# yuliangguo/OmniFusion

Measured on AMD Instinct MI355X. Metric: panoramas/sec at 512x1024 ERP, N=18 256^2 patches; equi2pers+pers2equi GB/s vs HBM peak, higher is better.
Workload: dtype f16x3 (fp16 hi/lo pairs, fp32 accumulate: fp32-class); 1 GPU; cfg2/cfg4 shard: 8 panoramas/GPU/step, 512x1024 ERP, fov 80, nrows 4 (18 patches); full single-pass spherical_fusion forward (confidence=True) at patch size 128 — the only size the reference network exists at (SURVEY 0.1); random-init weights (seed 42); inputs resident in HBM; resample pair at 18x256^2 reported in roofline_resample; per_gpu_batch=8, global_batch=8, parallelism=image-sharded x1, execution=3 forwards in flight per GPU on 3 streams (spherical_fusion.pipelined)

## Files before the change

omnifusion_amd/csrc/omni_conv_sh.hip:

```cpp
#include "omni_conv_sh_common.h"

namespace {

__constant__ float wino_coef[16][4] = {
    {1, 0, 0, 0}, {1, 1, 0, 0}, {1, -1, 0, 0}, {0, -1, 0, 0},
    {1, 0, 1, 0}, {1, 1, 1, 1}, {1, -1, 1, -1}, {0, -1, 0, -1},
    {1, 0, -1, 0}, {1, 1, -1, -1}, {1, -1, -1, 1}, {0, -1, 0, 1},
    {0, 0, -1, 0}, {0, 0, -1, -1}, {0, 0, -1, 1}, {0, 0, 0, 1}};
template <int BM, int BN, int WM, int WN, int NST = 3, int NL = 0, bool PP = false, bool WINO = false, bool X1 = false>
__global__ __launch_bounds__(64 * (WM * WN + NL)) void conv_sh_kernel(ShConvArgs a)
{
    static_assert(!(WINO && X1), "Winograd: f16x3 only");
    static_assert(!PP || (NL > 0 && WM * WN == 8 && NST >= 3), "ping-pong: eight matrix waves (two per SIMD) + loader waves, three stages");
    static_assert(!WINO || (PP && BM / WM == 32 && BN / WN == 32), "Winograd: the ping-pong kernel with 32 x 32 wave tiles");
    constexpr int NW = WM * WN, LW = NL > 0 ? NL : NW, RPP = 8 * LW;
    constexpr int TM = BM / WM / 32, TN = BN / WN / 32;
    constexpr int APASS = BM / RPP, BPASS = BN / RPP, LPS = APASS + BPASS;
    static_assert(APASS >= 1 && BPASS >= 1, "a tile side must cover at least one DMA pass");
    constexpr int A_BYTES = BM * 128, STAGE = (BM + BN) * 128;
    __shared__ __attribute__((aligned(1024))) unsigned char lds[NST * STAGE];
    __shared__ long long cst[OMNI_ABL(32768) ? 256 : 1];
    const bool stamped = OMNI_ABL(32768) && blockIdx.x == 0 && blockIdx.y == 0 && a.ws != nullptr && a.splitk <= 1;
    auto cstamp = [&](int k) { if (OMNI_ABL(32768) && stamped && (threadIdx.x & 63) == 0 && k < 256) cst[k] = clock64(); };
    auto cdump = [&]() { if (OMNI_ABL(32768) && stamped && threadIdx.x == 0) for (int i = 0; i < 256; ++i) reinterpret_cast<long long*>(a.ws)[i] = cst[i]; };
// ... 498 lines not shown
                                       const void* res, void* dst, int fmt, int M, int H, int W, int C1, int C2, int Cout,
                                       int KH, int KW, int stride, int pad, int act, int splitk, float* ws, size_t ws_bytes,
                                       omni_stream_t stream)
{
    return conv2d_sh_impl(src1, src2, wt16, bias, res, dst, fmt, M, H, W, C1, C2, Cout, KH, KW, stride, pad, act, splitk, ws, ws_bytes,
                          nullptr, 0, stream);
}
extern "C" int omni_conv2d_sh_f16x3_post_ws(const void* src1, const void* src2, const void* wt16, const float* bias,
                                            const void* res, void* dst, int fmt, int M, int H, int W, int C1, int C2, int Cout,
                                            int KH, int KW, int stride, int pad, int act, int splitk, float* ws, size_t ws_bytes,
                                            const float* post, size_t post_elems, omni_stream_t stream)
{
    return conv2d_sh_impl(src1, src2, wt16, bias, res, dst, fmt, M, H, W, C1, C2, Cout, KH, KW, stride, pad, act, splitk, ws, ws_bytes,
                          post, post_elems, stream);
}
extern "C" int omni_gemm_sh_f16x3_ln512_ws(const void* x, const void* wt16, const float* bias, const float* res, float* tok, const float* ln_g, const float* ln_b,
                                           float eps, void* y, int fmt, int rows, int K, int splitk, float* ws, size_t ws_bytes, omni_stream_t stream)
{
    if (!x || !wt16 || !tok || !ln_g || !ln_b || !y) OMNI_FAIL(OMNI_ERR_INVALID, "omni_gemm_sh_f16x3_ln512: null pointer");
    if (rows <= 0 || K <= 0 || K % 32) OMNI_FAIL(OMNI_ERR_INVALID, "omni_gemm_sh_f16x3_ln512: bad shape");
    if (fmt & 8) OMNI_FAIL(OMNI_ERR_UNSUPPORTED, "omni_gemm_sh_f16x3_ln512: no f16x1 form (fmt bit 3)");
    const int S = std::min(splitk, K / 32);
    if (S < 2) OMNI_FAIL(OMNI_ERR_INVALID, "omni_gemm_sh_f16x3_ln512: needs a split-K plan (splitk >= 2); an unsplit GEMM writes its result in its own epilogue");
    const int rc = conv2d_sh_impl(x, nullptr, wt16, bias, res, tok, 2, rows, 1, 1, K, 0, 512, 1, 1, 1, 0, OMNI_ACT_NONE, S, ws, ws_bytes, nullptr, 0, stream, false);
    if (rc != OMNI_OK) return rc;
    hipStream_t s = (hipStream_t)stream;
    if (fmt & 1) hipLaunchKernelGGL(sh_splitk_reduce_ln512_kernel<true>, dim3((rows + 3) / 4), dim3(256), 0, s, (const float*)ws, bias, res, tok, ln_g, ln_b, y, rows, S, (size_t)rows * 512, eps);
    else         hipLaunchKernelGGL(sh_splitk_reduce_ln512_kernel<false>, dim3((rows + 3) / 4), dim3(256), 0, s, (const float*)ws, bias, res, tok, ln_g, ln_b, y, rows, S, (size_t)rows * 512, eps);
    OMNI_HIP(hipGetLastError());
    return OMNI_OK;
}

constexpr int OMNI_HALO2_MIN_BLOCKS = 256;
template <bool X1>
static void conv_sh_select(const ShConvArgs& a, int fmt, hipStream_t s)
{
    const int KH = a.KH, KW = a.KW, stride = a.stride, pad = a.pad, H = a.H, W = a.W, M = a.M, Cout = a.Cout;
    const int ksteps = KH * KW * ((a.C1 + a.C2) / 32);
    const long long rows = a.rows;
    if (const int h2 = omni_options().conv_halo2; h2 > 0 && a.splitk <= 1 && KH == 3 && KW == 3 && stride == 1 && pad == 1 && Cout % 64 == 0 && rows % 256 == 0 &&
        !(fmt & 4) && !omni_options().conv_nohalo && omni_options().conv_halo_bn != 32) {
        const int iw = (H == 16 && W == 16 && omni_options().conv_img > 0) ? 16 : (W % HT_W == 0 && H % 8 == 0) ? 0 : -1;
        const long long blocks = (rows / 256) * (Cout / 64);
        if (iw >= 0 && (h2 == 2 || blocks >= (h2 == 1 ? OMNI_HALO2_MIN_BLOCKS : h2))) { omni_halo2_launch(&a, iw, X1, s); return; }
    }
    if (a.splitk <= 1 && KH == 3 && KW == 3 && stride == 1 && pad == 1 && H == W && (W == 16 || (W == 8 && omni_options().conv_img >= 2)) && rows % 128 == 0 &&
        Cout % 64 == 0 && !(fmt & 4) && omni_options().conv_img > 0 && !omni_options().conv_nohalo) {
        const int grid = (int)(rows / 128) * (Cout / 64);
        if (omni_options().conv_halo_bn == 32) {
            if (W == 16) omni_halo_launch(&a, 32, 4, false, 16, X1, 2 * grid, s);
            else         omni_halo_launch(&a, 32, 4, false, 8, X1, 2 * grid, s);
        }
        else if (W == 16) omni_halo_launch(&a, 64, 4, false, 16, X1, grid, s);
        else         omni_halo_launch(&a, 64, 4, false, 8, X1, grid, s);
        return;
    }
    if (a.splitk <= 1 && KH == 3 && KW == 3 && stride == 1 && pad == 1 && W % HT_W == 0 && H % 4 == 0 && !omni_options().conv_nohalo) {
        const int th = (H % 8 == 0 && omni_options().conv_halo_th == 8) ? 8 : 4;
        const int grid = M * (H / th) * (W / HT_W);
        if (th == 8) {
            if (Cout % 64 == 0 && omni_options().conv_halo_bn != 32) omni_halo_launch(&a, 64, 8, false, 0, X1, grid * (Cout / 64), s);
            else                omni_halo_launch(&a, 32, 8, false, 0, X1, grid * (Cout / 32), s);
        } else {
            const bool bn32 = omni_options().conv_halo_bn == 32 || ((fmt & 4) && omni_options().conv_halo_bn_lat == 32);
            if (Cout % 64 == 0 && !bn32) omni_halo_launch(&a, 64, 4, false, 0, X1, grid * (Cout / 64), s);
            else                omni_halo_launch(&a, 32, 4, false, 0, X1, grid * (Cout / 32), s);
        }
        return;
    }
    int tile = omni_options().conv_sh_tile;
    if (tile < 0) tile = 8;
    const int pm = omni_options().conv_pm;
    const bool pm_shape = pm > 0 && KH == 3 && KW == 3 && stride == 1 && pad == 1 && H == W && (W == 8 || W == 4) && Cout % 64 == 0 && !a.post &&
                          omni_options().conv_pingpong && !(pm == 3 && W != 8) && !(pm == 4 && W != 4);
    if (pm_shape && pm == 2) { omni_conv_pm_launch(&a, Cout % 128 == 0 ? 128 : 64, X1, s); return; }
    const bool big256 = tile == 8 && Cout % 128 == 0 && ((rows + 255) / 256) * (long long)(Cout / 128) * a.splitk >= std::max(1, omni_options().conv_big_blocks);
    if (pm_shape && tile == 8 && !big256) {
        if (Cout % 128 == 0 && ((rows + 127) / 128) * (long long)(Cout / 128) * a.splitk >= 128) { omni_conv_pm_launch(&a, 128, X1, s); return; }
        if (((rows + 127) / 128) * (long long)(Cout / 64) * a.splitk >= 128) { omni_conv_pm_launch(&a, 64, X1, s); return; }
    }
    if (Cout % 64 != 0) launch_sh<X1, 128, 32, 4, 1>(a, s);
    else if (tile == 2 && Cout % 128 == 0) launch_sh<X1, 128, 128, 2, 2>(a, s);
    else if (tile == 1) launch_sh<X1, 128, 64, 2, 2>(a, s);
    else if (tile == 3) launch_sh<X1, 128, 64, 4, 2>(a, s);
    else if (tile == 4 && Cout % 128 == 0) launch_sh<X1, 128, 128, 4, 2>(a, s);
    else if (tile == 8 && Cout % 128 == 0 && ((rows + 255) / 256) * (long long)(Cout / 128) * a.splitk >= std::max(1, omni_options().conv_big_blocks)) launch_sh<X1, 256, 128, 4, 2>(a, s);
    else if (tile == 8 && Cout % 128 == 0 && ((rows + 127) / 128) * (long long)(Cout / 128) * a.splitk >= 128) launch_sh<X1, 128, 128, 4, 2, 3, 4>(a, s);
    else if (tile == 8 && ((rows + 127) / 128) * (long long)(Cout / 64) * a.splitk >= 128) launch_sh<X1, 128, 64, 4, 2, 3, 4>(a, s);
    else if (tile == 9 && Cout % 128 == 0 && ((rows + 255) / 256) * (long long)(Cout / 128) * a.splitk >= 128) launch_sh<X1, 256, 128, 4, 2>(a, s);
// ... 52 lines not shown
    hipStream_t s = (hipStream_t)stream;
    if (fmt & 8) conv_sh_select<true>(a, fmt, s);
    else         conv_sh_select<false>(a, fmt, s);
    OMNI_HIP(hipGetLastError());
    if (a.splitk > 1 && reduce) {
        const size_t n4 = (size_t)rows * Cout / 4;
        hipLaunchKernelGGL(sh_splitk_reduce_kernel, dim3((unsigned)((n4 + 255) / 256)), dim3(256), 0, s, (const float*)ws, bias, res, dst,
                           n4, Cout, a.splitk, (size_t)rows * Cout, act, a.dst_sh, a.res_f32);
        OMNI_HIP(hipGetLastError());
    }
    return OMNI_OK;
}

extern "C" int omni_splitk_reduce_ln512(const float* parts, int nparts, const float* bias, const float* res, float* tok, const float* lg, const float* lb,
                                        float eps, void* y, int fmt, int rows, omni_stream_t stream)
{
    if (!parts || nparts < 1 || !tok || !lg || !lb || !y || rows <= 0) OMNI_FAIL(OMNI_ERR_INVALID, "omni_splitk_reduce_ln512: null pointer or empty input");
    hipStream_t s = (hipStream_t)stream;
    if (fmt & 1) hipLaunchKernelGGL(sh_splitk_reduce_ln512_kernel<true>, dim3((rows + 3) / 4), dim3(256), 0, s, parts, bias, res, tok, lg, lb, y, rows, nparts, (size_t)rows * 512, eps);
    else         hipLaunchKernelGGL(sh_splitk_reduce_ln512_kernel<false>, dim3((rows + 3) / 4), dim3(256), 0, s, parts, bias, res, tok, lg, lb, y, rows, nparts, (size_t)rows * 512, eps);
    OMNI_HIP(hipGetLastError());
    return OMNI_OK;
}

OMNI_SH_OVERFLOW_ACCESSOR(omni_sh_overflow_conv)

extern "C" int omni_sh_overflow(int* flag, int reset)
{
    if (!flag) OMNI_FAIL(OMNI_ERR_INVALID, "omni_sh_overflow: null output");
    OMNI_HIP(hipDeviceSynchronize());
    unsigned v = 0;
    if (omni_sh_overflow_conv(&v, reset) != 0 || omni_sh_overflow_halo(&v, reset) != 0 || omni_sh_overflow_up2(&v, reset) != 0 ||
        omni_sh_overflow_rows(&v, reset) != 0 || omni_sh_overflow_net(&v, reset) != 0 || omni_sh_overflow_pm(&v, reset) != 0 ||
        omni_sh_overflow_halo2(&v, reset) != 0)
        OMNI_FAIL(OMNI_ERR_HIP, "omni_sh_overflow: could not read the device flag");
    *flag = v ? 1 : 0;
    return OMNI_OK;
}

extern "C" int omni_sh_from_f32(const float* src, void* dst, size_t n, omni_stream_t stream)
{
    if (!src || !dst || n % 32) OMNI_FAIL(OMNI_ERR_INVALID, "omni_sh_from_f32: null pointer or n % 32 != 0");
    if (n == 0) return OMNI_OK;
    hipLaunchKernelGGL(sh_from_f32_kernel, dim3((unsigned)((n / 4 + 255) / 256)), dim3(256), 0, (hipStream_t)stream, src, dst, n / 4);
    OMNI_HIP(hipGetLastError());
    return OMNI_OK;
}
extern "C" int omni_sh_to_f32(const void* src, float* dst, size_t n, omni_stream_t stream)
{
    if (!src || !dst || n % 32) OMNI_FAIL(OMNI_ERR_INVALID, "omni_sh_to_f32: null pointer or n % 32 != 0");
    if (n == 0) return OMNI_OK;
    hipLaunchKernelGGL(sh_to_f32_kernel, dim3((unsigned)((n / 4 + 255) / 256)), dim3(256), 0, (hipStream_t)stream, src, dst, n / 4);
    OMNI_HIP(hipGetLastError());
    return OMNI_OK;
}

namespace {

__global__ __launch_bounds__(256) void wino_input_sh_kernel(const void* __restrict__ src, void* __restrict__ V, int M, int H, int W, int C, size_t nt)
{
    const size_t i = (size_t)blockIdx.x * 256 + threadIdx.x;
    const int cq = C >> 2;
    if (i >= nt * cq) return;
    const size_t tl = i / cq;
    const int c = (int)(i - tl * cq) * 4;
    const int tw = W >> 1, th = H >> 1;
    const int m = (int)(tl / (size_t)(th * tw)), rem = (int)(tl - (size_t)m * th * tw), ty = rem / tw, tx = rem - ty * tw;
// ... 63 lines not shown
```

omnifusion_amd/csrc/omni_conv_sh_common.h:

```cpp
#pragma once
#include <stdlib.h>
#include <algorithm>
#include <type_traits>
#include "omni_internal.h"
#include "omni_sh.h"

#ifndef OMNI_CONV_ABL
#define OMNI_CONV_ABL 0
#endif
#define OMNI_ABL(bit) ((OMNI_CONV_ABL & (bit)) != 0)
#ifndef OMNI_PP_PRIO
#define OMNI_PP_PRIO 0
#endif
#ifndef OMNI_G1_PW
#define OMNI_G1_PW 4
#endif

namespace {

typedef float f16v __attribute__((ext_vector_type(16)));
typedef float f4v __attribute__((ext_vector_type(4)));
typedef _Float16 h8v __attribute__((ext_vector_type(8)));
typedef _Float16 h4v __attribute__((ext_vector_type(4)));
typedef _Float16 h2v __attribute__((ext_vector_type(2)));
// ... 171 lines not shown

__device__ __forceinline__ void splitk_finish(f4v v, size_t o, const float* __restrict__ bias, const void* __restrict__ res, void* __restrict__ dst,
                                              int Cout, int act, int dst_sh, int res_f32)
{
    if (bias) v += *reinterpret_cast<const f4v*>(bias + (o % Cout));
    if (res && res_f32) v += *reinterpret_cast<const f4v*>((const float*)res + o);
    else if (res) {
        const unsigned char* rp = (const unsigned char*)res + sh_off(o);
        v += sh_join4(*reinterpret_cast<const h4v*>(rp), *reinterpret_cast<const h4v*>(rp + 64));
    }
    if (act == OMNI_ACT_RELU) { v.x = fmaxf(v.x, 0.f); v.y = fmaxf(v.y, 0.f); v.z = fmaxf(v.z, 0.f); v.w = fmaxf(v.w, 0.f); }
    else if (act == OMNI_ACT_GELU) {
#pragma unroll
        for (int e = 0; e < 4; ++e) v[e] = 0.5f * v[e] * (1.0f + erff(v[e] * 0.70710678118654752440f));
    }
    if (dst_sh) {
        h4v hi, lo; sh_split4(v, hi, lo);
        unsigned char* dp = (unsigned char*)dst + sh_off(o);
        *reinterpret_cast<h4v*>(dp) = hi; *reinterpret_cast<h4v*>(dp + 64) = lo;
    } else {
        *reinterpret_cast<f4v*>((float*)dst + o) = v;
    }
}

constexpr int HT_W = 32, HPW = HT_W + 2;

}

void omni_halo_launch(const void* args, int bn, int th, bool up2, int iw, bool x1, unsigned grid, hipStream_t s);
void omni_conv_pm_launch(const void* args, int bn, bool x1, hipStream_t s);
int omni_sh_overflow_pm(unsigned* out, int reset);
void omni_halo2_launch(const void* args, int iw, bool x1, hipStream_t s);
int omni_sh_overflow_halo2(unsigned* out, int reset);
int omni_sh_overflow_halo(unsigned* out, int reset);
int omni_sh_overflow_up2(unsigned* out, int reset);
int omni_sh_overflow_rows(unsigned* out, int reset);
int omni_sh_overflow_net(unsigned* out, int reset);
```

omnifusion_amd/csrc/omni_conv_up2.hip:

```cpp
#include "omni_conv_sh_common.h"

namespace {

constexpr int HR_PITCH = 36;
struct HeadsArgs { const void* w16; float* hr; };

template <bool HEADS, bool X1 = false>
__global__ __launch_bounds__(HEADS ? 64 * (4 + OMNI_G1_PW) : 512) void conv3x3_up2_g1_kernel(ShConvArgs a, int ntiles, HeadsArgs hd)
{
    constexpr int BN = 32, TH = 4, NW = 4, RPP = 8 * NW;
    constexpr int PW = HEADS ? OMNI_G1_PW : 4, CPT = 32 / PW;
    constexpr int HPX = (TH + 2) * HPW, HA_INSTR = (HPX * 8 + 63) / 64, HA_BYTES = HA_INSTR * 1024;
    constexpr int BROWS = 3 * BN, BPASS = (BROWS + RPP - 1) / RPP, B_BYTES = BROWS * 128, W_OFF = 2 * HA_BYTES;
    __shared__ __attribute__((aligned(1024))) unsigned char lds[2 * HA_BYTES + 3 * B_BYTES];
    constexpr int ST_N = 40, ST_K = 5;
    __shared__ long long stamps[OMNI_ABL(32768) ? 2 * ST_N * ST_K : 1];
    auto stamp = [&](int who, int it, int k) { if (OMNI_ABL(32768) && blockIdx.x == 0 && it < ST_N && (threadIdx.x & 63) == 0) stamps[(who * ST_N + it) * ST_K + k] = clock64(); };

    const int t = threadIdx.x, lane = t & 63;
    const int wave = __builtin_amdgcn_readfirstlane(t >> 6);
    const bool consumer = wave < NW;
    const int tw = a.W / HT_W, th = a.H / TH, per_img = tw * th;
    const int xcd = blockIdx.x & 7, lb = blockIdx.x >> 3, nlb = gridDim.x >> 3;
    const int per = (ntiles + 7) >> 3, t_end = min(ntiles, (xcd + 1) * per);
// ... 266 lines not shown
}

}

OMNI_SH_OVERFLOW_ACCESSOR(omni_sh_overflow_up2)

extern "C" int omni_conv3x3_up2_sh_f16x3(const void* src, const void* wt16, const float* bias, void* dst, int fmt,
                                         int M, int Hl, int Wl, int C, int Cout, int act, omni_stream_t stream)
{
    if (!src || !wt16 || !dst) OMNI_FAIL(OMNI_ERR_INVALID, "omni_conv3x3_up2_sh: null pointer");
    if (M <= 0 || Hl <= 0 || Wl <= 0 || C <= 0 || C % 32 || Cout <= 0 || Cout % 32) OMNI_FAIL(OMNI_ERR_INVALID, "omni_conv3x3_up2_sh: bad shape (channels must be multiples of 32)");
    const int H = 2 * Hl, W = 2 * Wl;
    if (W % HT_W || H % 4) OMNI_FAIL(OMNI_ERR_UNSUPPORTED, "omni_conv3x3_up2_sh: the output must be a multiple of 4 rows x 32 columns");
    if ((long long)M * H * W >= (1ll << 31) || (long long)Cout * 9 * C * 4 >= (1ll << 31))
        OMNI_FAIL(OMNI_ERR_UNSUPPORTED, "omni_conv3x3_up2_sh: tensor too large for 32-bit indices");
    ShConvArgs a;
    a.src1 = src; a.src2 = nullptr; a.wt = wt16; a.bias = bias; a.res = nullptr; a.dst = dst; a.dst_sh = fmt & 1; a.res_f32 = 0;
    a.dbg = 0; a.noxcd = omni_options().conv_noxcd; a.wt_major = 0; a.epi_lds = omni_options().conv_epi_lds && !(fmt & 4);
#ifdef OMNI_DEBUG_BUILD
    a.dbg = omni_debug_bits("OMNI_CONV_DBG");
#endif
    a.M = M; a.H = H; a.W = W; a.C1 = C; a.C2 = 0; a.Cout = Cout; a.KH = 3; a.KW = 3; a.stride = 1; a.pad = 1; a.act = act;
    a.Ho = H; a.Wo = W; a.rows = M * H * W; a.splitk = 1; a.ws = nullptr; a.post = nullptr; a.post_rows = 1; a.wino_th = a.wino_tw = a.wino_pix = 0;
    const int grid = M * (H / 4) * (W / HT_W);
    const bool x1 = (fmt & 8) != 0;
    if (C == 32 && Cout == 32 && omni_options().conv_up2_persist) {
        const dim3 g1(grid < 256 ? (grid + 7) / 8 * 8 : 256);
        if (x1) hipLaunchKernelGGL((conv3x3_up2_g1_kernel<false, true>), g1, dim3(512), 0, (hipStream_t)stream, a, grid, HeadsArgs{nullptr, nullptr});
        else    hipLaunchKernelGGL(conv3x3_up2_g1_kernel<false>, g1, dim3(512), 0, (hipStream_t)stream, a, grid, HeadsArgs{nullptr, nullptr});
        OMNI_HIP(hipGetLastError());
        return OMNI_OK;
    }
    const bool bn64 = Cout % 64 == 0 && !((fmt & 4) && omni_options().conv_halo_up2_bn_lat == 32);
    if (bn64) omni_halo_launch(&a, 64, 4, true, 0, x1, grid * (Cout / 64), (hipStream_t)stream);
    else      omni_halo_launch(&a, 32, 4, true, 0, x1, grid * (Cout / 32), (hipStream_t)stream);
    OMNI_HIP(hipGetLastError());
    return OMNI_OK;
}

extern "C" size_t omni_up2_heads_scratch_bytes(int M, int P)
{
    if (M <= 0 || P <= 0 || P % 32) return 0;
    return (size_t)M * (P / 4) * (P / 32) * 4 * 6 * HR_PITCH * sizeof(float);
}
template <bool X1>
static int up2_heads_impl(const void* src, const void* wt16, const float* bias, const void* heads_w16f, float bias_pred, float bias_weight,
                          float* scratch, size_t scratch_bytes, float* out_a, float* out_c, int M, int P, int confidence, omni_stream_t stream)
{
    if (!src || !wt16 || !heads_w16f || !scratch || !out_a) OMNI_FAIL(OMNI_ERR_INVALID, "omni_conv3x3_up2_heads_sh: null pointer");
    if (M <= 0 || P <= 0 || P % 32) OMNI_FAIL(OMNI_ERR_INVALID, "omni_conv3x3_up2_heads_sh: the patch size must be a multiple of 32");
    if (scratch_bytes < omni_up2_heads_scratch_bytes(M, P)) OMNI_FAIL(OMNI_ERR_INVALID, "omni_conv3x3_up2_heads_sh: scratch too small (omni_up2_heads_scratch_bytes)");
    if ((long long)M * P * P >= (1ll << 31)) OMNI_FAIL(OMNI_ERR_UNSUPPORTED, "omni_conv3x3_up2_heads_sh: tensor too large for 32-bit indices");
    ShConvArgs a;
    a.src1 = src; a.src2 = nullptr; a.wt = wt16; a.bias = bias; a.res = nullptr; a.dst = nullptr; a.dst_sh = 0; a.res_f32 = 0;
    a.dbg = 0; a.noxcd = omni_options().conv_noxcd; a.wt_major = 0; a.epi_lds = 0;
    a.M = M; a.H = P; a.W = P; a.C1 = 32; a.C2 = 0; a.Cout = 32; a.KH = 3; a.KW = 3; a.stride = 1; a.pad = 1; a.act = OMNI_ACT_RELU;
    a.Ho = P; a.Wo = P; a.rows = M * P * P; a.splitk = 1; a.ws = nullptr; a.post = nullptr; a.post_rows = 1; a.wino_th = a.wino_tw = a.wino_pix = 0;
    const int grid = M * (P / 4) * (P / HT_W);
    hipLaunchKernelGGL((conv3x3_up2_g1_kernel<true, X1>), dim3(grid < 256 ? (grid + 7) / 8 * 8 : 256), dim3(64 * (4 + OMNI_G1_PW)), 0, (hipStream_t)stream, a, grid, HeadsArgs{heads_w16f, scratch});
    OMNI_HIP(hipGetLastError());
    const size_t n = (size_t)M * P * P / 4;
    hipLaunchKernelGGL(heads_finish_kernel, dim3((unsigned)((n + 255) / 256)), dim3(256), 0, (hipStream_t)stream, (const float*)scratch, bias_pred, bias_weight,
                       out_a, out_c, M, P, confidence);
    OMNI_HIP(hipGetLastError());
    return OMNI_OK;
}
extern "C" int omni_conv3x3_up2_heads_sh_f16x3(const void* src, const void* wt16, const float* bias, const void* heads_w16f, float bias_pred, float bias_weight,
// ... 30 lines not shown
```

omnifusion_amd/csrc/omni_geometry.hip:

```cpp
#include <math.h>
#include <stdlib.h>
#include <string.h>
#include <mutex>
#include <vector>
#include <memory>

#include "omni_internal.h"

static thread_local std::string g_err;
void omni_set_error(const std::string& msg) { g_err = msg; }
extern "C" const char* omni_last_error(void) { return g_err.c_str(); }
extern "C" int omni_version(void) { return OMNI_VERSION; }

namespace {
struct OptName { const char* name; const char* env; int OmniOptions::* field; int dflt; };
const OptName kOpts[] = {
    {"conv_sh_tile", "OMNI_CONV_SH_TILE", &OmniOptions::conv_sh_tile, -1},
    {"conv_nohalo", "OMNI_CONV_NOHALO", &OmniOptions::conv_nohalo, 0},
    {"conv_halo_th", "OMNI_CONV_HALO_TH", &OmniOptions::conv_halo_th, 4},
    {"conv_big_blocks", "OMNI_CONV_BIG_BLOCKS", &OmniOptions::conv_big_blocks, 128},
    {"conv_halo_bn_lat", "OMNI_CONV_HALO_BN_LAT", &OmniOptions::conv_halo_bn_lat, 32},
    {"conv_deep_loaders", "OMNI_CONV_DEEP_LOADERS", &OmniOptions::conv_deep_loaders, 1},
    {"conv_halo_up2_bn_lat", "OMNI_CONV_HALO_UP2_BN_LAT", &OmniOptions::conv_halo_up2_bn_lat, 64},
    {"conv_halo_bn", "OMNI_CONV_HALO_BN", &OmniOptions::conv_halo_bn, 64},
// ... 11 lines not shown
    {"e2p_notab", "OMNI_E2P_NOTAB", &OmniOptions::e2p_notab, 0},
    {"e2p_verbose", "OMNI_E2P_VERBOSE", &OmniOptions::e2p_verbose, 0},
    {"e2p_bwd_simple", "OMNI_E2P_BWD_SIMPLE", &OmniOptions::e2p_bwd_simple, 0},
    {"p2e_bwd_simple", "OMNI_P2E_BWD_SIMPLE", &OmniOptions::p2e_bwd_simple, 0},
    {"bwd_table_mb", "OMNI_BWD_TABLE_MB", &OmniOptions::bwd_table_mb, 1024},
    {"bwd_wide", "OMNI_BWD_WIDE", &OmniOptions::bwd_wide, 1},
    {"bwd_lmax", "OMNI_BWD_LMAX", &OmniOptions::bwd_lmax, 0},
    {"bwd_chunk", "OMNI_BWD_CHUNK", &OmniOptions::bwd_chunk, 0},
    {"p2e_gather", "OMNI_P2E_GATHER", &OmniOptions::p2e_gather, 0},
    {"e2p_nbuf", "OMNI_E2P_NBUF", &OmniOptions::e2p_nbuf, 0},
    {"e2p_slot_kb", "OMNI_E2P_SLOT_KB", &OmniOptions::e2p_slot_kb, 6},
    {"e2p_tile_h", "OMNI_E2P_TILE_H", &OmniOptions::e2p_tile_h, 0},
    {"e2p_ref_lds", "OMNI_E2P_REF_LDS", &OmniOptions::e2p_ref_lds, 1},
    {"e2p_store", "OMNI_E2P_STORE", &OmniOptions::e2p_store, 1},
    {"e2p_slots", "OMNI_E2P_SLOTS", &OmniOptions::e2p_slots, 0},
    {"e2p_split", "OMNI_E2P_SPLIT", &OmniOptions::e2p_split, 0},
    {"e2p_full", "OMNI_E2P_FULL", &OmniOptions::e2p_full, -1},
    {"e2p_fb_planes", "OMNI_E2P_FB_PLANES", &OmniOptions::e2p_fb_planes, 0},
    {"e2p_fb_pos", "OMNI_E2P_FB_POS", &OmniOptions::e2p_fb_pos, 0},
    {"e2p_region", "OMNI_E2P_REGION", &OmniOptions::e2p_region, 0},
    {"p2e_band", "OMNI_P2E_BAND", &OmniOptions::p2e_band, 0},
    {"p2e_nbuf", "OMNI_P2E_NBUF", &OmniOptions::p2e_nbuf, 0},
    {"p2e_lds_kb", "OMNI_P2E_LDS_KB", &OmniOptions::p2e_lds_kb, 0},
    {"p2e_planes", "OMNI_P2E_PLANES", &OmniOptions::p2e_planes, 0},
    {"p2e_walk", "OMNI_P2E_WALK", &OmniOptions::p2e_walk, 1},
    {"p2e_tile8", "OMNI_P2E_TILE8", &OmniOptions::p2e_tile8, 1},
    {"p2e_store", "OMNI_P2E_STORE", &OmniOptions::p2e_store, 1},
    {"fv_bwd_lds", "OMNI_FV_BWD_LDS", &OmniOptions::fv_bwd_lds, 1},
    {"geom_cache_max", "OMNI_GEOM_CACHE_MAX", &OmniOptions::geom_cache_max, 16},
    {"chamfer_split", "OMNI_CHAMFER_SPLIT", &OmniOptions::chamfer_split, 1},
    {"augment_lut", "OMNI_AUGMENT_LUT", &OmniOptions::augment_lut, 1},
    {"conv_halo2", "OMNI_CONV_HALO2", &OmniOptions::conv_halo2, 1},
    {"conv_wgrad_rows", "OMNI_CONV_WGRAD_ROWS", &OmniOptions::conv_wgrad_rows, 0},
};
}

OmniOptions& omni_options()
{
    static OmniOptions o = [] {
        OmniOptions v;
        for (const OptName& k : kOpts) {
            const char* e = getenv(k.env);
            v.*(k.field) = e ? (*e ? atoi(e) : 1) : k.dflt;
        }
        return v;
    }();
    return o;
}

int omni_num_cus()
{
    static int cus[64] = {0};
    int dev = 0;
    if (hipGetDevice(&dev) != hipSuccess || dev < 0 || dev >= 64) return 256;
    if (cus[dev] == 0) {
        int n = 0;
        cus[dev] = (hipDeviceGetAttribute(&n, hipDeviceAttributeMultiprocessorCount, dev) == hipSuccess && n > 0) ? n : 256;
    }
    return cus[dev];
}

extern "C" int omni_set_option(const char* name, int value)
{
    if (!name) OMNI_FAIL(OMNI_ERR_INVALID, "omni_set_option: null name");
    for (const OptName& k : kOpts)
        if (strcmp(k.name, name) == 0) { omni_options().*(k.field) = value; return OMNI_OK; }
// ... 235 lines not shown
```

omnifusion_amd/csrc/omni_internal.h:

```cpp
#pragma once
#include <mutex>
#include <hip/hip_runtime.h>
#include <hip/hip_fp16.h>
#include <stdint.h>
#include <string>
#include <vector>

#include "../../include/omnifusion.h"

#define OMNI_MAX_PATCH 46
#define OMNI_WAVE 64

void omni_set_error(const std::string& msg);
#define OMNI_FAIL(code, msg) do { omni_set_error(msg); return (code); } while (0)
#define OMNI_HIP(expr) do { hipError_t e_ = (expr); if (e_ != hipSuccess) {                   \
        omni_set_error(std::string(#expr) + ": " + hipGetErrorString(e_)); return OMNI_ERR_HIP; } } while (0)

struct OmniOptions {
    int conv_sh_tile;
    int conv_nohalo;
    int conv_halo_th;
    int conv_halo_bn_lat;
    int conv_halo_up2_bn_lat;
    int conv_deep_loaders;
// ... 13 lines not shown
    int e2p_notab;
    int e2p_verbose;
    int e2p_bwd_simple;
    int p2e_bwd_simple;
    int p2e_gather;
    int e2p_nbuf;
    int e2p_store;
    int e2p_slots;
    int e2p_split;
    int e2p_full;
    int e2p_fb_planes;
    int e2p_region;
    int e2p_fb_pos;
    int e2p_ref_lds;
    int e2p_tile_h;
    int e2p_slot_kb;
    int p2e_band;
    int p2e_lds_kb;
    int p2e_nbuf;
    int p2e_planes;
    int p2e_store;
    int p2e_tile8;
    int p2e_walk;
    int bwd_wide;
    int bwd_chunk;
    int bwd_lmax;
    int bwd_table_mb;
    int fv_bwd_lds;
    int geom_cache_max;
    int chamfer_split;
    int augment_lut;
    int conv_halo2;
    int conv_wgrad_rows;
};
OmniOptions& omni_options();
int omni_num_cus();

#ifdef OMNI_DEBUG_BUILD
#define OMNI_DBG(a, bit) (((a).dbg & (bit)) != 0)
int omni_debug_bits(const char* env_name);
long long* omni_debug_trace_buf();
#else
#define OMNI_DBG(a, bit) false
#endif

struct PatchTab {
    int   N;
    float lam0[OMNI_MAX_PATCH];
    float slam[OMNI_MAX_PATCH];
    float clam[OMNI_MAX_PATCH];
    float sphi[OMNI_MAX_PATCH];
    float cphi[OMNI_MAX_PATCH];
};

constexpr int OMNI_SP_LMAX = 48;
struct OmniSpTable {
    uint2* ent = nullptr; int* slice_off = nullptr; int* cnt = nullptr;
    uint2* long_ent = nullptr; int* long_off = nullptr; int* long_row = nullptr;
    int nrows = 0, nslices = 0, nlong = 0, ok = 0;
    long long nent = 0, npadded = 0, nlong_ent = 0;
};
void omni_sp_free(OmniSpTable& t);
struct omni_geometry;
int omni_bwd_workspace(omni_geometry* g, hipStream_t stream, size_t bytes, float** out);

struct omni_geometry {
// ... 79 lines not shown
```

omnifusion_amd/isa.py:

```python
import os
import re
import subprocess
import sys
import tempfile

LLVM = os.environ.get("OMNI_LLVM_BIN", "/opt/rocm/lib/llvm/bin")
TARGET = "hipv4-amdgcn-amd-amdhsa--gfx950"
FORBIDDEN = re.compile(r"\bv_pk_(mul|add|fma)_f32\b")
COUNTED = ("e2p_box_kernel", "p2e_lds_kernel", "p2e_walk_kernel", "e2p_ref_kernel")
HOT = ("conv_sh_kernel", "conv3x3_halo_sh_kernel", "conv3x3_up2_g1_kernel", "stem_f16x3_pc_kernel", "heads_kernel", "maxpool_kernel",
       "layernorm512_kernel", "attention_kernel", "upsample_sh8_kernel", "halo2_sh_kernel")
HOST_ONLY = ("omni_png.o", "omni_geometry.o")


def _device_object(obj, tmp):
    fat = os.path.join(tmp, "fat.bin")
    co = os.path.join(tmp, "dev.co")
    r = subprocess.run([os.path.join(LLVM, "llvm-objcopy"), "--dump-section", f".hip_fatbin={fat}", obj, os.path.join(tmp, "copy.o")],
                       stderr=subprocess.DEVNULL)
    if r.returncode != 0 or not os.path.exists(fat) or os.path.getsize(fat) == 0:
        return None
    subprocess.check_call([os.path.join(LLVM, "clang-offload-bundler"), "--unbundle", "--type=o", f"--input={fat}",
                           f"--targets={TARGET}", f"--output={co}"])
    return co


def disassemble(obj):
    with tempfile.TemporaryDirectory() as tmp:
        co = _device_object(obj, tmp)
        if co is None:
            return ""
        return subprocess.check_output([os.path.join(LLVM, "llvm-objdump"), "-d", "--mcpu=gfx950", co]).decode()


def kernel_meta(obj):
    with tempfile.TemporaryDirectory() as tmp:
        co = _device_object(obj, tmp)
        if co is None:
            return []
        txt = subprocess.check_output([os.path.join(LLVM, "llvm-readelf"), "--notes", co]).decode()
    out, cur = [], None
    keys = {".vgpr_count": "vgpr", ".agpr_count": "agpr", ".sgpr_count": "sgpr", ".group_segment_fixed_size": "lds",
            ".private_segment_fixed_size": "scratch", ".vgpr_spill_count": "vgpr_spill", ".sgpr_spill_count": "sgpr_spill",
            ".name": "name"}
# ... 88 lines not shown
```

Measured before the change: 4362 panoramas/s.

## Add 8-row halo conv kernel with fused 2x bilinear upsampling and 32-wide form

Adds a new 3x3 convolution kernel that covers 8 output rows per block. It stages the haloed input tile once per channel group in LDS and streams weights through a four-slot ring. One variant builds the upsampled input tile directly in LDS from the half-resolution source, using bilinear interpolation split into fp16 hi/lo parts. The other variant handles Cout not divisible by 64 with 32-channel tiles. Both are enabled by default through a new option and are chosen when the existing halo2 block-count heuristic allows. The aim is to raise input reuse and to avoid materialising the upsampled tensor, at the cost of more LDS and register pressure, fewer blocks, and extra interpolation math inside the kernel.

```diff
diff --git a/omnifusion_amd/csrc/omni_conv_halo2x.hip b/omnifusion_amd/csrc/omni_conv_halo2x.hip
--- /dev/null
+++ b/omnifusion_amd/csrc/omni_conv_halo2x.hip
@@ -0,0 +1,270 @@
+#include <stdio.h>
+#include <string.h>
+#include "omni_conv_sh_common.h"
+
+namespace {
+
+template <int BN, bool UP2, bool X1>
+__global__ __launch_bounds__(256, 2) void halo2x_sh_kernel(ShConvArgs a)
+{
+    static_assert((BN == 64 && UP2) || (BN == 32 && !UP2), "the up-sampling form with 64 channels per block, the copying form with 32");
+    constexpr int TN = BN / 32, NW = 4, RPP = 8 * NW, RING = 4, TROWS = 8;
+    constexpr int HPX = (TROWS + 2) * HPW, HA_INSTR = (HPX * 8 + 63) / 64, HA_BYTES = HA_INSTR * 1024;
+    constexpr int APASS = (HA_INSTR + NW - 1) / NW, BPASS = BN / RPP, B_BYTES = BN * 128;
+    constexpr int CROWS = (TROWS + 2) / 2, CCOLS = HPW / 2, UTASKS = CROWS * CCOLS * 4;
+    static_assert(UTASKS > 256 && UTASKS <= 384, "one pass of four waves and one of two");
+    __shared__ __attribute__((aligned(1024))) unsigned char lds[HA_BYTES + RING * B_BYTES];
+    static_assert(sizeof(lds) <= 80 * 1024, "two blocks per CU");
+
+    const int t = threadIdx.x, lane = t & 63;
+    const int wave = __builtin_amdgcn_readfirstlane(t >> 6);
+    const int ntn = a.Cout / BN, tw = a.W / HT_W, th = a.H / TROWS;
+    int bid = a.noxcd ? blockIdx.x : omni_xcd_remap(blockIdx.x, gridDim.x);
+    const int tile_n = bid % ntn; bid /= ntn;
+    const int tx = bid % tw; bid /= tw;
+    const int ty = bid % th; const int m = bid / th;
+    const int y0 = ty * TROWS, x0 = tx * HT_W, col0 = tile_n * BN;
+    const int G1 = a.C1 >> 5, G = (a.C1 + a.C2) >> 5, ksteps = 9 * G;
+
+    const int gs = (lane & 15) ^ ((4 * wave + (lane >> 4)) & 15);
+    const int rl = 8 * wave + 2 * (lane >> 4) + (gs >> 3), pc16 = (gs & 7) * 16;
+    int wbase[BPASS];
+#pragma unroll
+    for (int i = 0; i < BPASS; ++i) wbase[i] = (col0 + rl + RPP * i) * ksteps * 128 + pc16;
+    const rsrc_t rsw = make_rsrc(a.wt, (size_t)a.Cout * ksteps * 128);
+
+    [[maybe_unused]] auto issue_a = [&](int g) {
+        const rsrc_t rs1 = make_rsrc(a.src1, (size_t)a.M * a.H * a.W * a.C1 * 4);
+        const rsrc_t rs2 = make_rsrc(a.src2 ? a.src2 : a.src1, a.src2 ? (size_t)a.M * a.H * a.W * a.C2 * 4 : 0);
+        const bool first = g < G1;
+        const int cs4 = (first ? a.C1 : a.C2) * 4;
+        const int soff = (first ? g : g - G1) * 128 + pc16;
+        unsigned char* sb = lds + wave * 1024;
+        int rlv = rl;
+        asm volatile("" : "+v"(rlv));
+#pragma unroll
+        for (int i = 0; i < APASS; ++i) {
+            if (wave + NW * i < HA_INSTR) {
+                const int p = rlv + RPP * i, hy = p / HPW, hx = p - hy * HPW;
+                const int iy = y0 - 1 + hy, ix = x0 - 1 + hx;
+                const int px = (p < HPX && (unsigned)iy < (unsigned)a.H && (unsigned)ix < (unsigned)a.W) ? (m * a.H + iy) * a.W + ix : -1;
+                const int off = px >= 0 ? px * cs4 + soff : (int)0x80000000;
+                if (first) dma16(rs1, sb + i * (1024 * NW), off, 0);
+                else       dma16(rs2, sb + i * (1024 * NW), off, 0);
+            }
+        }
+    };
+
+    [[maybe_unused]] auto up_load = [&](int g, int task, h8v (&ch)[4], h8v (&cl)[4]) {
+        const int Hl = a.H >> 1, Wl = a.W >> 1;
+        const int u_c8 = task & 3, u_cell = task >> 2, u_ci = u_cell / CCOLS, u_cj = u_cell - u_ci * CCOLS;
+        const int u_k = (y0 >> 1) - 1 + u_ci, u_j = (x0 >> 1) - 1 + u_cj;
+        const int ra = min(max(u_k, 0), Hl - 1), rb = min(max(u_k + 1, 0), Hl - 1), ca = min(max(u_j, 0), Wl - 1), cb = min(max(u_j + 1, 0), Wl - 1);
+        const size_t pp = (size_t)a.C1 * 4, img = (size_t)m * Hl * Wl;
+        const unsigned char* sp = (const unsigned char*)a.src1 + (size_t)g * 128 + u_c8 * 16;
+        const size_t u_src[4] = {(img + (size_t)ra * Wl + ca) * pp, (img + (size_t)ra * Wl + cb) * pp, (img + (size_t)rb * Wl + ca) * pp, (img + (size_t)rb * Wl + cb) * pp};
+#pragma unroll
+        for (int q = 0; q < 4; ++q) { ch[q] = *reinterpret_cast<const h8v*>(sp + u_src[q]); cl[q] = *reinterpret_cast<const h8v*>(sp + u_src[q] + 64); }
+    };
+    [[maybe_unused]] auto up_put = [&](int task, const h8v (&ch)[4], const h8v (&cl)[4]) {
+        const int u_c8 = task & 3, u_cell = task >> 2, u_ci = u_cell / CCOLS, u_cj = u_cell - u_ci * CCOLS;
+        const int u_k = (y0 >> 1) - 1 + u_ci, u_j = (x0 >> 1) - 1 + u_cj;
+        float u_ly[2], u_lx[2];
+        bool u_in[2][2];
+#pragma unroll
+        for (int d = 0; d < 2; ++d) {
+            const int oy = 2 * u_k + 1 + d, ox = 2 * u_j + 1 + d;
+            const float fy = fmaxf(0.5f * ((float)oy + 0.5f) - 0.5f, 0.0f), fx = fmaxf(0.5f * ((float)ox + 0.5f) - 0.5f, 0.0f);
+            u_ly[d] = fy - (float)(int)fy; u_lx[d] = fx - (float)(int)fx;
+        }
+#pragma unroll
+        for (int dy = 0; dy < 2; ++dy)
+#pragma unroll
+            for (int dx = 0; dx < 2; ++dx)
+                u_in[dy][dx] = (unsigned)(2 * u_k + 1 + dy) < (unsigned)a.H && (unsigned)(2 * u_j + 1 + dx) < (unsigned)a.W;
+        float v[4][8];
+#pragma unroll
+        for (int q = 0; q < 4; ++q)
+#pragma unroll
+            for (int e = 0; e < 8; ++e) v[q][e] = fmaf((float)cl[q][e], 4.8828125e-4f, (float)ch[q][e]);
+#pragma unroll
+        for (int dy = 0; dy < 2; ++dy)
+#pragma unroll
+            for (int dx = 0; dx < 2; ++dx) {
+                const float ly = u_ly[dy], lx = u_lx[dx], hy = 1.0f - ly, hx = 1.0f - lx;
+                h8v oh, ol;
+#pragma unroll
+                for (int e = 0; e < 8; ++e) {
+                    const float o = hy * (hx * v[0][e] + lx * v[1][e]) + ly * (hx * v[2][e] + lx * v[3][e]);
+                    const _Float16 hh = (fabsf(o) < 6.103515625e-05f) ? (_Float16)0.0f : (_Float16)o;
+                    oh[e] = u_in[dy][dx] ? hh : (_Float16)0.0f;
+                    ol[e] = u_in[dy][dx] ? (_Float16)((o - (float)hh) * 2048.0f) : (_Float16)0.0f;
+                }
+                const int p = (2 * u_ci + dy) * HPW + 2 * u_cj + dx, d = p >> 1, pc = (p & 1) * 8 + u_c8;
+                *reinterpret_cast<h8v*>(lds + d * 256 + ((pc ^ (d & 15)) * 16)) = oh;
+                *reinterpret_cast<h8v*>(lds + d * 256 + (((pc + 4) ^ (d & 15)) * 16)) = ol;
+            }
+    };
+    [[maybe_unused]] auto fill_a = [&](int g, bool sync) {
+        int tv = t;
+        asm volatile("" : "+v"(tv));
+        h8v ch[4], cl[4];
+        up_load(g, tv, ch, cl);
+        if (sync) {
+            wait_lds_reads();
+            __builtin_amdgcn_s_barrier();
+            asm volatile("" ::: "memory");
+        }
+        up_put(tv, ch, cl);
+        if (wave < 2) {
+            int tu = t + 256;
+            asm volatile("" : "+v"(tu));
+            if (tu < UTASKS) {
+                h8v dh[4], dl[4];
+                up_load(g, tu, dh, dl);
+                up_put(tu, dh, dl);
+            }
+        }
+    };
+    auto issue_b = [&](int g, int tap, int slot) {
+        unsigned char* sb = lds + HA_BYTES + slot * B_BYTES + wave * 1024;
+        const int soff = (tap * G + g) * 128;
+#pragma unroll
+        for (int i = 0; i < BPASS; ++i) dma16(rsw, sb + i * (1024 * NW), wbase[i], soff);
+    };
+
+    int ao[4][3];
+#pragma unroll
+    for (int r = 0; r < 4; ++r)
+#pragma unroll
+        for (int kx = 0; kx < 3; ++kx) {
+            const int q = (2 * wave + r) * HPW + (lane & 31) + kx;
+            const int d = q >> 1;
+            ao[r][kx] = d * 256 + ((((q & 1) * 8 + (lane >> 5)) ^ (d & 15)) * 16);
+        }
+    int fo[4];
+    {
+        const int r = lane & 31, v = r >> 1, h = lane >> 5;
+#pragma unroll
+        for (int k = 0; k < 4; ++k) fo[k] = v * 256 + ((((r & 1) * 8 + 2 * k + h) ^ v) * 16);
+    }
+
+    f16v acc[2][TN], acc1[2][TN];
+#pragma unroll
+    for (int p = 0; p < 2; ++p)
+#pragma unroll
+        for (int j = 0; j < TN; ++j) { acc[p][j] = (f16v)(0.0f); acc1[p][j] = (f16v)(0.0f); }
+    h8v kh[3][2], kl[3][2];
+
+    if constexpr (UP2) { issue_b(0, 0, 0); issue_b(0, 1, 1); issue_b(0, 2, 2); fill_a(0, false); }
+    else               { issue_a(0); issue_b(0, 0, 0); issue_b(0, 1, 1); issue_b(0, 2, 2); }
+    int T = 0;
+    for (int g = 0; g < G; ++g) {
+#pragma unroll
+        for (int tap = 0; tap < 9; ++tap) {
+            const int ky = tap / 3, kx = tap - 3 * ky;
+            if (tap == 0 || T + 1 >= ksteps) wait_vm<0>();
+            else if (T + 2 >= ksteps) wait_vm<BPASS>();
+            else wait_vm<2 * BPASS>();
+            wait_lds_reads();
+            __builtin_amdgcn_s_barrier();
+            asm volatile("" ::: "memory");
+            if (T + 3 < ksteps) {
+                if (tap + 3 < 9) issue_b(g, tap + 3, (T + 3) & 3);
+                else             issue_b(g + 1, tap + 3 - 9, (T + 3) & 3);
+            }
+            const unsigned char* sB = lds + HA_BYTES + (T & 3) * B_BYTES;
+            int a_old = ao[0][kx], a_new = ao[ky + 1][kx];
+            asm volatile("" : "+v"(a_old), "+v"(a_new));
+#pragma unroll
+            for (int kc = 0; kc < 2; ++kc) {
+                if (ky == 0) {
+                    kh[kx][kc] = *reinterpret_cast<const h8v*>(lds + (a_old ^ (kc * 32)));
+                    if constexpr (!X1) kl[kx][kc] = *reinterpret_cast<const h8v*>(lds + (a_old ^ (64 + kc * 32)));
+                }
+                const h8v nh = *reinterpret_cast<const h8v*>(lds + (a_new ^ (kc * 32)));
+                h8v nl;
+                if constexpr (!X1) nl = *reinterpret_cast<const h8v*>(lds + (a_new ^ (64 + kc * 32)));
+#pragma unroll
+                for (int j = 0; j < TN; ++j) {
+                    const unsigned char* bp = sB + j * 32 * 128;
+                    const h8v bh = *reinterpret_cast<const h8v*>(bp + fo[kc]);
+                    h8v bl;
+                    if constexpr (!X1) bl = *reinterpret_cast<const h8v*>(bp + fo[2 + kc]);
+                    acc[0][j] = __builtin_amdgcn_mfma_f32_32x32x16_f16(bh, kh[kx][kc], acc[0][j], 0, 0, 0);
+                    if constexpr (!X1) {
+                        acc1[0][j] = __builtin_amdgcn_mfma_f32_32x32x16_f16(bl, kh[kx][kc], acc1[0][j], 0, 0, 0);
+                        acc1[0][j] = __builtin_amdgcn_mfma_f32_32x32x16_f16(bh, kl[kx][kc], acc1[0][j], 0, 0, 0);
+                    }
+                    acc[1][j] = __builtin_amdgcn_mfma_f32_32x32x16_f16(bh, nh, acc[1][j], 0, 0, 0);
+                    if constexpr (!X1) {
+                        acc1[1][j] = __builtin_amdgcn_mfma_f32_32x32x16_f16(bl, nh, acc1[1][j], 0, 0, 0);
+                        acc1[1][j] = __builtin_amdgcn_mfma_f32_32x32x16_f16(bh, nl, acc1[1][j], 0, 0, 0);
+                    }
+                }
+                kh[kx][kc] = nh;
+                if constexpr (!X1) kl[kx][kc] = nl;
+            }
+            ++T;
+        }
+        if (g + 1 < G) {
+            if constexpr (UP2) fill_a(g + 1, true);
+            else {
+                wait_lds_reads();
+                __builtin_amdgcn_s_barrier();
+                asm volatile("" ::: "memory");
+                issue_a(g + 1);
+            }
+        }
+    }
+
+    int c0[TN];
+#pragma unroll
+    for (int j = 0; j < TN; ++j) c0[j] = col0 + j * 32;
+    size_t r0[2], r1[2];
+#pragma unroll
+    for (int p = 0; p < 2; ++p) { r0[p] = ((size_t)m * a.H + y0 + 2 * wave + p) * a.W + x0; r1[p] = r0[p] + 16; }
+    if (a.dst_sh && !a.res_f32 && a.epi_lds) {
+        static_assert(NW * 32 * (32 * TN + 4) * 4 <= (int)sizeof(lds), "the transposition tiles must fit the K loop's buffers");
+        wait_lds_reads();
+        __syncthreads();
+        float* tile = reinterpret_cast<float*>(lds) + wave * (32 * (32 * TN + 4));
+#pragma unroll
+        for (int p = 0; p < 2; ++p) {
+            epilogue_tile_lds<TN, true, X1>(acc[p], acc1[p], a, r0[p], 32, c0, lane, tile, r1[p]);
+            asm volatile("s_waitcnt lgkmcnt(0)" ::: "memory");
+        }
+        return;
+    }
+#pragma unroll
+    for (int p = 0; p < 2; ++p) {
+        const size_t r = ((lane & 31) < 16 ? r0[p] : r1[p]) + (lane & 15);
+#pragma unroll
+        for (int j = 0; j < TN; ++j) {
+            const f16v ea[1] = {acc[p][j]}, eb[1] = {acc1[p][j]};
+            const int cj[1] = {c0[j]};
+            epilogue_row<1, 2, X1>(ea, eb, a, r, cj, lane, a.dst_sh != 0);
+        }
+    }
+}
+
+}
+
+OMNI_SH_OVERFLOW_ACCESSOR(omni_sh_overflow_halo2x)
+
+void omni_halo2x_launch(const void* args, bool up2, bool x1, hipStream_t s)
+{
+    ShConvArgs a;
+    memcpy(&a, args, sizeof(a));
+    const bool shape = a.KH == 3 && a.KW == 3 && a.stride == 1 && a.pad == 1 && a.splitk <= 1 && a.W % HT_W == 0 && a.H % 8 == 0 && a.rows % 256 == 0 &&
+                       (up2 ? (a.Cout % 64 == 0 && a.C2 == 0) : a.Cout % 32 == 0);
+    if (!shape) {
+        fprintf(stderr, "omni_halo2x_launch: no halo2x_sh_kernel<up2 %d> for %d x %d x %d, %d -> %d channels\n", (int)up2, a.M, a.H, a.W, a.C1 + a.C2, a.Cout);
+        abort();
+    }
+    const dim3 grid((unsigned)(a.rows / 256) * (unsigned)(a.Cout / (up2 ? 64 : 32))), block(256);
+    if (up2 && !x1) hipLaunchKernelGGL((halo2x_sh_kernel<64, true, false>), grid, block, 0, s, a);
+    else if (up2)   hipLaunchKernelGGL((halo2x_sh_kernel<64, true, true>), grid, block, 0, s, a);
+    else if (!x1)   hipLaunchKernelGGL((halo2x_sh_kernel<32, false, false>), grid, block, 0, s, a);
+    else            hipLaunchKernelGGL((halo2x_sh_kernel<32, false, true>), grid, block, 0, s, a);
+}
diff --git a/omnifusion_amd/csrc/omni_conv_sh.hip b/omnifusion_amd/csrc/omni_conv_sh.hip
--- a/omnifusion_amd/csrc/omni_conv_sh.hip
+++ b/omnifusion_amd/csrc/omni_conv_sh.hip
@@ -554,6 +554,15 @@
 }
 
 constexpr int OMNI_HALO2_MIN_BLOCKS = 256;
+bool omni_halo2x_take(int form, long long blocks, int fmt)
+{
+    const OmniOptions& o = omni_options();
+    const int d = (form == 0 ? o.conv_halo2x : o.conv_halo2x / 10) % 10;
+    if (d <= 0 || (fmt & 4) || o.conv_nohalo || o.conv_halo_bn == 32 || o.conv_halo_th == 8) return false;
+    if (d >= 2) return true;
+    const int h2 = o.conv_halo2;
+    return h2 == 2 || (h2 > 0 && blocks >= (h2 == 1 ? OMNI_HALO2_MIN_BLOCKS : h2));
+}
 template <bool X1>
 static void conv_sh_select(const ShConvArgs& a, int fmt, hipStream_t s)
 {
@@ -577,6 +586,8 @@
         else         omni_halo_launch(&a, 64, 4, false, 8, X1, grid, s);
         return;
     }
+    if (a.splitk <= 1 && KH == 3 && KW == 3 && stride == 1 && pad == 1 && W % HT_W == 0 && H % 8 == 0 && Cout % 64 != 0 &&
+        omni_halo2x_take(1, (rows / 256) * (Cout / 32), fmt)) { omni_halo2x_launch(&a, false, X1, s); return; }
     if (a.splitk <= 1 && KH == 3 && KW == 3 && stride == 1 && pad == 1 && W % HT_W == 0 && H % 4 == 0 && !omni_options().conv_nohalo) {
         const int th = (H % 8 == 0 && omni_options().conv_halo_th == 8) ? 8 : 4;
         const int grid = M * (H / th) * (W / HT_W);
@@ -695,7 +706,7 @@
     unsigned v = 0;
     if (omni_sh_overflow_conv(&v, reset) != 0 || omni_sh_overflow_halo(&v, reset) != 0 || omni_sh_overflow_up2(&v, reset) != 0 ||
         omni_sh_overflow_rows(&v, reset) != 0 || omni_sh_overflow_net(&v, reset) != 0 || omni_sh_overflow_pm(&v, reset) != 0 ||
-        omni_sh_overflow_halo2(&v, reset) != 0)
+        omni_sh_overflow_halo2(&v, reset) != 0 || omni_sh_overflow_halo2x(&v, reset) != 0)
         OMNI_FAIL(OMNI_ERR_HIP, "omni_sh_overflow: could not read the device flag");
     *flag = v ? 1 : 0;
     return OMNI_OK;
diff --git a/omnifusion_amd/csrc/omni_conv_sh_common.h b/omnifusion_amd/csrc/omni_conv_sh_common.h
--- a/omnifusion_amd/csrc/omni_conv_sh_common.h
+++ b/omnifusion_amd/csrc/omni_conv_sh_common.h
@@ -227,6 +227,9 @@
 int omni_sh_overflow_pm(unsigned* out, int reset);
 void omni_halo2_launch(const void* args, int iw, bool x1, hipStream_t s);
 int omni_sh_overflow_halo2(unsigned* out, int reset);
+void omni_halo2x_launch(const void* args, bool up2, bool x1, hipStream_t s);
+int omni_sh_overflow_halo2x(unsigned* out, int reset);
+bool omni_halo2x_take(int form, long long blocks, int fmt);
 int omni_sh_overflow_halo(unsigned* out, int reset);
 int omni_sh_overflow_up2(unsigned* out, int reset);
 int omni_sh_overflow_rows(unsigned* out, int reset);
diff --git a/omnifusion_amd/csrc/omni_conv_up2.hip b/omnifusion_amd/csrc/omni_conv_up2.hip
--- a/omnifusion_amd/csrc/omni_conv_up2.hip
+++ b/omnifusion_amd/csrc/omni_conv_up2.hip
@@ -322,7 +322,8 @@
         return OMNI_OK;
     }
     const bool bn64 = Cout % 64 == 0 && !((fmt & 4) && omni_options().conv_halo_up2_bn_lat == 32);
-    if (bn64) omni_halo_launch(&a, 64, 4, true, 0, x1, grid * (Cout / 64), (hipStream_t)stream);
+    if (bn64 && H % 8 == 0 && omni_halo2x_take(0, (long long)(a.rows / 256) * (Cout / 64), fmt)) omni_halo2x_launch(&a, true, x1, (hipStream_t)stream);
+    else if (bn64) omni_halo_launch(&a, 64, 4, true, 0, x1, grid * (Cout / 64), (hipStream_t)stream);
     else      omni_halo_launch(&a, 32, 4, true, 0, x1, grid * (Cout / 32), (hipStream_t)stream);
     OMNI_HIP(hipGetLastError());
     return OMNI_OK;
diff --git a/omnifusion_amd/csrc/omni_geometry.hip b/omnifusion_amd/csrc/omni_geometry.hip
--- a/omnifusion_amd/csrc/omni_geometry.hip
+++ b/omnifusion_amd/csrc/omni_geometry.hip
@@ -67,6 +67,7 @@
     {"augment_lut", "OMNI_AUGMENT_LUT", &OmniOptions::augment_lut, 1},
     {"conv_halo2", "OMNI_CONV_HALO2", &OmniOptions::conv_halo2, 1},
     {"conv_wgrad_rows", "OMNI_CONV_WGRAD_ROWS", &OmniOptions::conv_wgrad_rows, 0},
+    {"conv_halo2x", "OMNI_CONV_HALO2X", &OmniOptions::conv_halo2x, 1},
 };
 }
 
diff --git a/omnifusion_amd/csrc/omni_internal.h b/omnifusion_amd/csrc/omni_internal.h
--- a/omnifusion_amd/csrc/omni_internal.h
+++ b/omnifusion_amd/csrc/omni_internal.h
@@ -69,6 +69,7 @@
     int augment_lut;
     int conv_halo2;
     int conv_wgrad_rows;
+    int conv_halo2x;
 };
 OmniOptions& omni_options();
 int omni_num_cus();
diff --git a/omnifusion_amd/isa.py b/omnifusion_amd/isa.py
--- a/omnifusion_amd/isa.py
+++ b/omnifusion_amd/isa.py
@@ -9,7 +9,7 @@
 FORBIDDEN = re.compile(r"\bv_pk_(mul|add|fma)_f32\b")
 COUNTED = ("e2p_box_kernel", "p2e_lds_kernel", "p2e_walk_kernel", "e2p_ref_kernel")
 HOT = ("conv_sh_kernel", "conv3x3_halo_sh_kernel", "conv3x3_up2_g1_kernel", "stem_f16x3_pc_kernel", "heads_kernel", "maxpool_kernel",
-       "layernorm512_kernel", "attention_kernel", "upsample_sh8_kernel", "halo2_sh_kernel")
+       "layernorm512_kernel", "attention_kernel", "upsample_sh8_kernel", "halo2_sh_kernel", "halo2x_sh_kernel")
 HOST_ONLY = ("omni_png.o", "omni_geometry.o")
 
 
```

Measured after the change: 4390 panoramas/s, median of 6. About the same (+0.6%).
